# eyedealism/flexible-LLM-sharding

Measured on AMD Instinct MI355X. Metric: tokens/sec + peak GPU mem, Llama-2-70B layer_num_per_shard=1 at 1/2/4/8 MI355X, higher is better.
Workload: dtype fp16

## Files before the change

csrc/include/fls.h:

```cpp
#pragma once
#include <stdint.h>
#include <stddef.h>

#ifdef __cplusplus
extern "C" {
#endif

typedef void* fls_stream_t;

int   fls_rt_version(void);
void* fls_pinned_alloc(uint64_t bytes);
int   fls_pinned_free(void* p);
void* fls_host_device_ptr(void* p);
int   fls_pinned_register(void* p, uint64_t bytes);
int   fls_pinned_unregister(void* p);
int   fls_memcpy_async(void* dst, const void* src, uint64_t bytes, int kind, fls_stream_t s);
int64_t fls_pread_into(const char* path, uint64_t offset, uint64_t bytes, void* dst, int nthreads);
int64_t fls_pwrite_from(const char* path, uint64_t offset, uint64_t bytes, const void* src,
                        int nthreads, int truncate);
int   fls_gather_blocks(void* dst, const void* src, uint64_t block_bytes, const int64_t* src_block,
                        int64_t n_blocks, int nthreads);
void* fls_st_open(const char* path);
int   fls_st_count(void* h);
int   fls_st_info(void* h, int i, char* name, int name_cap, char* dtype, int dtype_cap,
// ... 31 lines not shown
             const float* sin_t, int rope_cols, int head_dim, const void* bias, const float* rscale,
             float alpha, float* ss, int ss_ld, void* ws, uint64_t ws_bytes,
             fls_stream_t s);
int fls_row_stat(const void* x, int ldx, int rows, int H, float eps, float* rstd, fls_stream_t s);
int fls_row_ss(const void* x, int ldx, int rows, int H, float* ss, int ss_ld, fls_stream_t s);
int fls_rstd_from_ss(const float* ss, int ss_ld, int nparts, int rows, int H, float eps, float* rstd,
                     fls_stream_t s);
int fls_argmax_rows(const void* x, int ld, int rows, int V, int* out, fls_stream_t s);
int fls_row_rstd(const void* x, int ldx, const int* row_idx, int rows, int H, float eps, float* rstd,
                 fls_stream_t s);
int fls_fold_norm(void* w, int ldw, int N, int K, const void* gamma, fls_stream_t s);
int fls_copy_d2d(void* dst, const void* src, uint64_t bytes, int mode, int blocks, fls_stream_t s);
int fls_copy_rows(const void* x, int ldx, const int* src_idx, void* y, int ldy, const int* dst_idx, int rows, int H,
                  fls_stream_t s);
int fls_gemm_set_splitk(int on);
int fls_gemm_set_row_chunk(int rows);
int fls_moe_route(const void* logits, int ldl, int T, int E, int k, int norm, int round16, int* ids, float* w,
                  fls_stream_t s);
int fls_moe_router_route(const void* h, int ldh, const void* wr, int ldw, int T, int H, int E, int k, int norm,
                         int round16, int* ids, float* w, fls_stream_t s);
int fls_moe_plan_scratch(int n, int E);
int fls_moe_plan(const int* ids, int n, int k, int E, int* offs, int* tiles, int* rows, int* dest, int* bhist,
                 fls_stream_t s);
int fls_moe_gemm(const void* A, const void* W, void* C, int M_bound, int N, int K, int lda, int ldw, int ldc, int epi,
                 const int* tiles, const int* offs, const int* rows, int n_groups, long long wstride, int a_rows,
                 fls_stream_t s);
int fls_moe_combine(const void* y, int ldy, const int* ids, const int* dest, const float* w, void* x, int ldx, int T,
                    int k, int H, const void* sh, int ldsh, fls_stream_t s);
int fls_gemm_set_order(int order);
int fls_gemm_set_mid_bn(int bn);
int fls_gemm_set_mid_waves(int waves);
int fls_gemm_set_mid_rows(int rows);
int fls_gemm_set_mid(int on);
int fls_attention_set_hpb(int hpb);
int fls_attention_set_split(int ns);
int fls_attention_set_persistent(int on);
int fls_attention(const void* qkv, void* out, const int* work, int n_items, int n_q_heads,
                  int n_kv_heads, int head_dim, int ld_qkv, int ld_out, float scale, const void* kv0,
                  int ld_kv0, const int* seg_lo, int q_block, const int* work2, const int* r2win,
                  void* ws, unsigned long long ws_bytes, int n_rows, fls_stream_t s);
int fls_attention_window(const void* qkv, void* out, const int* work, int n_items, int n_q_heads,
                         int n_kv_heads, int head_dim, int ld_qkv, int ld_out, float scale, const void* kv0,
                         int ld_kv0, const int* seg_lo, int q_block, const int* work2, const int* r2win,
                         void* ws, unsigned long long ws_bytes, int n_rows, const int* r0_lo,
                         const int* r0_item, fls_stream_t s);
int fls_headnorm_rope(void* x, int ldx, int rows, int n_q, int n_k, const void* qn, const void* kn, const int* pos,
                      const float* cos_t, const float* sin_t, int hd, float eps, fls_stream_t s);
int fls_rmsnorm(const void* x, const void* w, void* y, const int* row_idx, int rows, int H,
                int ldx, int ldy, float eps, fls_stream_t s);
int fls_embed(const int* ids, const void* table, void* out, int T, int H, int V, float scale, fls_stream_t s);
int fls_softmax_rows(const void* logits, void* probs, int rows, int V, float inv_scale, fls_stream_t s);
int fls_logprob_rows(const void* logits, int ld, int rows, int V, const int* targets, float inv_scale, float* out,
                     fls_stream_t s);
int fls_sample_rows(const void* probs, int ld, int rows, int V, const uint32_t* table, const uint64_t* draws,
                    int top_k, int P, int* out, fls_stream_t s);
int fls_topk_rows(const void* probs, int ld, int rows, int V, int K, int* ids, void* vals, const int* picked,
                  void* picked_vals, fls_stream_t s);
int fls_verify_rows(const void* probs, int ld, int rows, int V, const int* row_start, int n_sfx, const int* draft,
                    int* tok, int* accept, int* keep, int* n_kept, fls_stream_t s);
int fls_pool_rows(const void* x, int ld, int n_src, int H, const int* row_idx, int n_list, const int* seg_start,
                  int n_seg, int D, int normalize, float* out, fls_stream_t s);
int fls_cast_f16(void* dst, const void* src, int src_dtype, uint64_t n, fls_stream_t s);
int fls_dequant_fp8(void* region, uint64_t n, const float* scale, int kind, uint64_t cols, fls_stream_t s);
int fls_dequant_fp8_launches(uint64_t n);
int fls_dequant_fp8_tail(void);
int fls_dequant_int4(void* region, uint64_t n, uint64_t group, int scale_dtype, fls_stream_t s);
// ... 12 lines not shown
```

csrc/kernels/gemm.hip:

```cpp
#include "gemm_v10.h"

namespace {

template <int EPI>
__global__ __launch_bounds__(256) void gemm_nt_generic(const half_t* __restrict__ A, const half_t* __restrict__ W,
                                                     half_t* __restrict__ C, int M, int N, int K, int lda, int ldw,
                                                     int ldc, Epi ep) {
  const int lane = threadIdx.x & 63, wave = threadIdx.x >> 6;
  const int fr = lane & 15, grp = lane >> 4;
  const int m0 = blockIdx.x * 32;
  const bool rope128 = EPI == FLS_EPI_ROPE;
  const int gbase = blockIdx.y * 256 + (wave >> 1) * 128;
  int ncol[4];
#pragma unroll
  for (int t = 0; t < 4; ++t) ncol[t] = gbase + sub_col(rope128, wave & 1, t);
  floatx4 acc[2][4];
#pragma unroll
  for (int u = 0; u < 2; ++u)
#pragma unroll
    for (int t = 0; t < 4; ++t) acc[u][t] = floatx4{0.f, 0.f, 0.f, 0.f};
  for (int k0 = 0; k0 < K; k0 += 32) {
    half8 wf[4], xf[2];
    const int kb = k0 + grp * 8;
#pragma unroll
// ... 478 lines not shown
    FLS_CHECK_LAUNCH();
    ss_partials(C, ldc, M, N, ep, s);
    FLS_CHECK_LAUNCH();
    return 0;
  }
  const int n_chunks = (M + ROW_CHUNK - 1) / ROW_CHUNK;
  const int step = ((M + n_chunks - 1) / n_chunks + BM - 1) / BM * BM;
  if (M > ROW_CHUNK && (size_t)(step / BM) * (N / BN) >= 256) {
    for (int r0 = 0; r0 < M; r0 += step) {
      Epi e = ep;
      if (e.pos) e.pos += r0;
      if (e.R) e.R += (size_t)r0 * e.ldr;
      if (e.ss) e.ss += (size_t)r0 * e.ss_ld;
      if (e.rs) e.rs += r0;
      const int rc = launch<EPI>(A + (size_t)r0 * lda, W, C + (size_t)r0 * ldc, min(step, M - r0), N, K, lda, ldw,
                                 ldc, e, s, ws, ws_bytes);
      if (rc) return rc;
    }
    return 0;
  }
  const int tiles = (int)tiles256;
  const int tiles_m = (M + BM - 1) / BM, tiles_n = N / BN;
  int order = g_order;
  if (order == 0) order = auto_order(tiles_m, tiles_n);
  Epi e = ep;
  e.order = order;
  launch_main<EPI>(tiles, A, W, C, M, N, K, lda, ldw, ldc, e, s);
  FLS_CHECK_LAUNCH();
  return 0;
}

}

extern "C" int fls_kernels_version(void) { return 40; }

extern "C" int fls_gemm_set_order(int order) {
  const int old = g_order;
  g_order = order;
  return old;
}

extern "C" int fls_gemm_set_skinny(int mode, int blocks) {
  const int old = g_skinny;
  g_skinny = mode < 0 ? 0 : mode > 2 ? 2 : mode;
  g_skinny_blocks = blocks > 0 ? blocks : 0;
  return old;
}

extern "C" int fls_gemm_set_skinny_bn(int bn) {
  const int old = g_skinny_bn;
  g_skinny_bn = bn == 128 || bn == 256 ? bn : 0;
  return old;
}

extern "C" int fls_gemm_set_splitk(int on) {
  const int old = g_splitk;
  g_splitk = on ? 1 : 0;
  return old;
}

extern "C" int fls_gemm_set_row_chunk(int rows) {
  const int old = ROW_CHUNK;
  ROW_CHUNK = rows > 0 ? rows : (1 << 30);
  return old;
}

extern "C" int fls_row_ss(const void* x, int ldx, int rows, int H, float* ss, int ss_ld, fls_stream_t s) {
// ... 84 lines not shown
```

csrc/kernels/gemm_v10.h:

```cpp
#pragma once
#include "common.h"
#include "fls.h"

#include <cstdlib>
#include <type_traits>

namespace {


constexpr int BM = 256, BN = 256, BK = 64;
constexpr int EPI_ROPE64 = 4;
constexpr int EPI_F32 = 6;
constexpr bool is_rope(int epi) { return epi == FLS_EPI_ROPE || epi == EPI_ROPE64; }
constexpr int BUF = 65536;
constexpr int WIMG = 32768;

struct Epi {
  const half_t* R;
  int ldr;
  const int* pos;
  const float* cos_t;
  const float* sin_t;
  int rope_cols;
  int head_dim;
  const half_t* bias;
  int gu_rows;
  int order;
  const int* g_tiles;
  const int* g_offs;
  const int* g_rows;
  long long g_wstride;
  int g_n;
  int ksplit;
  int kslice;
  long long part_stride;
  const float* rs = nullptr;
  float alpha = 1.f;
  float* ss = nullptr;
  int ss_ld = 0;
  int row_exact = 0;
};

__device__ __forceinline__ float row_sum_4groups(float v) {
// ... 203 lines not shown
    return;
  } else {
    const int off = 4 * grp;
    const int woff = wide_off(grp);
    if constexpr (EPI == FLS_EPI_SWIGLU) {
#pragma unroll
      for (int u = 0; u < U; ++u) {
        const int m = mrow0 + u * 16;
        const float s = ep.rs ? ep.rs[min(m, M - 1)] : 1.f;
        half4 o[4];
#pragma unroll
        for (int p = 0; p < 4; ++p)
#pragma unroll
          for (int r = 0; r < 4; ++r) o[p][r] = (half_t)(silu(acc[u][2 * p][r] * s) * (acc[u][2 * p + 1][r] * s));
#pragma unroll
        for (int p = 0; p < 4; p += 2) {
          const uint4 v = wide_pair(o[p], o[p + 1]);
          if (m < M && (!LO || m >= mlo)) *(uint4*)(C + (size_t)m * ldc + ncol0 / 2 + p * 16 + woff) = v;
        }
      }
      return;
    } else {
      half4 ba[4], bb[4];
#pragma unroll
      for (int p = 0; p < 4; ++p) {
        if (ep.bias) {
          ba[p] = *(const half4*)(ep.bias + ncol0 + p * 32 + off);
          bb[p] = *(const half4*)(ep.bias + ncol0 + p * 32 + off + 16);
        } else {
          ba[p] = half4{0, 0, 0, 0};
          bb[p] = half4{0, 0, 0, 0};
        }
      }
      uint4 rw[2][4];
      auto load = [&](int u, int sl) {
        if constexpr (EPI == FLS_EPI_RESID) {
          const int m = min(mrow0 + u * 16, M - 1);
          const half_t* rp = ep.R + (size_t)m * ep.ldr + ncol0 + woff;
#pragma unroll
          for (int p = 0; p < 4; ++p) rw[sl][p] = *(const uint4*)(rp + p * 32);
        }
      };
      float* const ssp = EPI == FLS_EPI_RESID ? ep.ss : nullptr;
      auto body = [&](auto has_bias) {
        load(0, 0);
#pragma unroll
        for (int u = 0; u < U; ++u) {
          const int sl = u & 1;
          if (u + 1 < U) load(u + 1, sl ^ 1);
          asm volatile("" ::: "memory");
          const int m = mrow0 + u * 16;
          const float s = ep.rs ? ep.rs[min(m, M - 1)] : 1.f;
          float sq = 0.f;
#pragma unroll
          for (int p = 0; p < 4; ++p) {
            floatx4 a = acc[u][2 * p] * s, b = acc[u][2 * p + 1] * s;
            if constexpr (decltype(has_bias)::value) {
#pragma unroll
              for (int r = 0; r < 4; ++r) { a[r] += (float)ba[p][r]; b[r] += (float)bb[p][r]; }
            }
            if constexpr (EPI == FLS_EPI_RESID) {
              half4 ra, rb;
              unwide_pair(rw[sl][p], ra, rb);
#pragma unroll
              for (int r = 0; r < 4; ++r) { a[r] = a[r] * ep.alpha + (float)ra[r]; b[r] = b[r] * ep.alpha + (float)rb[r]; }
            }
            half4 oa, ob;
#pragma unroll
            for (int r = 0; r < 4; ++r) { oa[r] = (half_t)a[r]; ob[r] = (half_t)b[r]; }
            if constexpr (EPI == FLS_EPI_RESID) {
              if (ssp) sq = ss_accum_pair(sq, oa, ob);
            }
            const uint4 v = wide_pair(oa, ob);
            if (m < M && (!LO || m >= mlo)) *(uint4*)(C + (size_t)m * ldc + ncol0 + p * 32 + woff) = v;
          }
          if constexpr (EPI == FLS_EPI_RESID) {
            if (ssp) {
              sq = row_sum_4groups(sq);
              if (grp == 0 && m < M && (!LO || m >= mlo)) ssp[(size_t)m * ep.ss_ld + (ncol0 >> 7)] = sq;
            }
          }
        }
// ... 239 lines not shown
```

csrc/kernels/gemm_v11.hip:

```cpp
#include "gemm_v10.h"


namespace {
namespace v11 {
constexpr int TM = 384, TN = 256, TK = 64;
constexpr int X01_0 = 0, X01_STG = 32768;
constexpr int X2_0 = 65536, X2_STG = 16384;
constexpr int W_0 = 98304, W_STG = 32768;
constexpr int LDS_BYTES = 163840;
}

__device__ __forceinline__ void mfma_acc_v_ordered(floatx4& c, const half8& a, const half8& b) {
  asm volatile("v_mfma_f32_16x16x32_f16 %0, %1, %2, %0" : "+v"(c) : "v"(a), "v"(b) : "memory");
}

template <int EPI>
__global__ __launch_bounds__(256, 1) void gemm_nt_v11(const half_t* __restrict__ A, const half_t* __restrict__ W,
                                                    half_t* __restrict__ C, int M, int N, int K, int lda, int ldw,
                                                    int ldc, Epi ep) {
  using namespace v11;
  extern __shared__ __attribute__((aligned(16))) char smem[];
  const int tid = threadIdx.x;
  const int lane = tid & 63;
  const int wave = __builtin_amdgcn_readfirstlane(tid >> 6);

  const int nwg = gridDim.x;
  int bid = blockIdx.x;
  {
    const int q = nwg >> 3, r = nwg & 7, xcd = bid & 7, loc = bid >> 3;
    bid = (xcd < r ? xcd * (q + 1) : r * (q + 1) + (xcd - r) * q) + loc;
  }
  const int tiles_m = (M + TM - 1) / TM;
  const int tiles_n = N / TN;
  const int2 tmn = tile_of(bid, tiles_m, tiles_n, ep.order);
  const int mlo = tmn.x * TM;
  const int m0 = min(mlo, M - TM);
  const int n0 = tmn.y * TN;

  const int lr = lane >> 3;
  const int lc = (lane & 7) ^ lr;
  const unsigned xl = (unsigned)(lr * lda + lc * 8) * 2u;
  const unsigned wl = (unsigned)(lr * ldw + lc * 8) * 2u;
  const char* Ab = (const char*)(A + (size_t)m0 * lda);
  const char* Wb = (const char*)(W + (size_t)(EPI == FLS_EPI_SWIGLU ? n0 / 2 : n0) * ldw);
  auto rsrc = [](const char* base, bool live) {
    return __builtin_amdgcn_make_buffer_rsrc(const_cast<char*>(base), (short)0, live ? -1 : 0, 0x00020000);
  };
  int xlds_p[3][4];
  unsigned xso[3][4];
#pragma unroll
  for (int j = 0; j < 3; ++j)
#pragma unroll
    for (int i = 0; i < 4; ++i) {
      const int p = 4 * wave + i;
      const int src_row = (p >> 3) * 192 + j * 64 + (p & 7) * 8;
      xlds_p[j][i] = j < 2 ? X01_0 + ((p >> 3) * 128 + j * 64 + (p & 7) * 8) * 128
                           : X2_0 + ((p >> 3) * 64 + (p & 7) * 8) * 128;
      xso[j][i] = (unsigned)(src_row * lda) * 2u;
    }
  unsigned wso[8];
#pragma unroll
  for (int i = 0; i < 8; ++i) {
    const int l = (8 * wave + i) * 8;
    const int pr = EPI == FLS_EPI_SWIGLU ? ((l >> 4) & 1) * ep.gu_rows + (l >> 5) * 16 + (l & 15) : l;
    wso[i] = (unsigned)(pr * ldw) * 2u;
  }
#define V11_DMA_X(rs, buf, j, i, k0)                                                               \
  __builtin_amdgcn_raw_ptr_buffer_load_lds(                                                        \
      rs, (LDS_AS void*)(smem + xlds_p[j][i] + (buf) * ((j) < 2 ? X01_STG : X2_STG)), 16, xl,      \
      xso[j][i] + (unsigned)(k0) * 2u, 0, 0)
#define V11_DMA_W(rs, buf, i, k0)                                                                  \
  __builtin_amdgcn_raw_ptr_buffer_load_lds(rs, (LDS_AS void*)(smem + W_0 + (buf) * W_STG + (8 * wave + (i)) * 1024), \
                                           16, wl, wso[i] + (unsigned)(k0) * 2u, 0, 0)

  const int wm = wave >> 1, wn = wave & 1;
  const int fr = lane & 15, grp = lane >> 4;
  const int sw = fr & 7;
  const int cs0 = ((0 + grp) ^ sw) << 4;
  const int cs1 = ((4 + grp) ^ sw) << 4;
  const int xrow = X01_0 + (wm * 128 + fr) * 128;
  const int x2row = X2_0 + (wm * 64 + fr) * 128;
  const int wrow = W_0 + (wn * 128 + fr) * 128;

  floatx4 acc[8][8], accv[4][8];
#pragma unroll
  for (int u = 0; u < 8; ++u)
#pragma unroll
    for (int t = 0; t < 8; ++t) acc[u][t] = floatx4{0.f, 0.f, 0.f, 0.f};
#pragma unroll
  for (int u = 0; u < 4; ++u)
#pragma unroll
    for (int t = 0; t < 8; ++t) accv[u][t] = floatx4{0.f, 0.f, 0.f, 0.f};
  half8 xf[12], wf[8];
#define V11_FENCE_ACC()                                                                            \
  _Pragma("unroll") for (int u_ = 0; u_ < 8; ++u_)                                                \
  _Pragma("unroll") for (int t_ = 0; t_ < 8; ++t_) asm volatile("" : "+a"(acc[u_][t_]));          \
  _Pragma("unroll") for (int u_ = 0; u_ < 4; ++u_)                                                \
  _Pragma("unroll") for (int t_ = 0; t_ < 8; ++t_) asm volatile("" : "+v"(accv[u_][t_]));
  V11_FENCE_ACC();
  asm volatile("s_nop 7\n\ts_nop 7" ::: "memory");

  const char* const bx01_0 = smem + xrow + cs0;
  const char* const bx01_1 = smem + xrow + cs1;
  const char* const bx2_0 = smem + x2row + cs0;
  const char* const bx2_1 = smem + x2row + cs1;
  const char* const bw_0 = smem + wrow + cs0;
  const char* const bw_1 = smem + wrow + cs1;
#define V11_RX(f, buf, s)                                                                          \
  xf[f] = (f) < 8 ? *(const half8*)(((s) ? bx01_1 : bx01_0) + (buf) * X01_STG + (f) * 2048)        \
                  : *(const half8*)(((s) ? bx2_1 : bx2_0) + (buf) * X2_STG + ((f) - 8) * 2048)
#define V11_RW(t, buf, s) wf[t] = *(const half8*)(((s) ? bw_1 : bw_0) + (buf) * W_STG + (t) * 2048)
#define V11_MFMA(u, t)                                                                             \
  do {                                                                                            \
    if ((u) < 8) mfma_acc_inplace_ordered(acc[(u) & 7][t], wf[t], xf[u]);                         \
    else mfma_acc_v_ordered(accv[(u) & 3][t], wf[t], xf[u]);                                      \
  } while (0)
#define V11_DMA_AT(i_, ND)                                                                         \
  ((ND) == 2 ? ((i_) == 9 ? 0 : (i_) == 21 ? 1 : -1)                                              \
   : (ND) == 4 ? ((i_) == 7 ? 0 : (i_) == 13 ? 1 : (i_) == 19 ? 2 : (i_) == 25 ? 3 : -1)          \
   : ((i_) == 5 ? 0 : (i_) == 9 ? 1 : (i_) == 13 ? 2 : (i_) == 17 ? 3 : (i_) == 21 ? 4 : (i_) == 25 ? 5 : -1))
#define V11_DMAS(i_, DMA_STMT, ND)                                                                 \
  {                                                                                               \
    const int d_ = V11_DMA_AT(i_, ND);                                                            \
    if (d_ >= 0) { DMA_STMT(d_); }                                                                \
  }
#define V11_SYNC(LGK, VMC)                                                                         \
  {                                                                                               \
    __builtin_amdgcn_s_waitcnt(0xC07F | ((LGK) << 8));                                            \
    asm volatile("s_waitcnt vmcnt(" #VMC ")" ::: "memory");                                       \
    __builtin_amdgcn_s_barrier();                                                                 \
  }

#define V11_PHASE_A(cbuf, cs, nbuf, ns, DMA_STMT, ND)                                             \
  _Pragma("unroll") for (int i_ = 0; i_ < 32; ++i_) {                                             \
    const int t_ = i_ >> 2, u_ = i_ & 3;                                                          \
    V11_MFMA(u_, t_);                                                                             \
    if (i_ == 1) V11_RX(8, cbuf, cs);                                                             \
    if (i_ == 3) V11_RX(9, cbuf, cs);                                                             \
    if (i_ >= 28) V11_RX(u_, nbuf, ns);                                                           \
    V11_DMAS(i_, DMA_STMT, ND);                                                                   \
  }
#define V11_PHASE_B(cbuf, cs, nbuf, ns, DMA_STMT, ND)                                             \
  _Pragma("unroll") for (int i_ = 0; i_ < 32; ++i_) {                                             \
    const int u_ = 4 + (i_ >> 3), t_ = i_ & 7;                                                    \
    V11_MFMA(u_, t_);                                                                             \
    if (i_ == 1) V11_RX(10, cbuf, cs);                                                            \
    if (i_ == 3) V11_RX(11, cbuf, cs);                                                            \
    if ((i_ & 7) == 7) V11_RX(u_, nbuf, ns);                                                      \
    V11_DMAS(i_, DMA_STMT, ND);                                                                   \
  }
#define V11_PHASE_C(nbuf, ns, DMA_STMT, ND)                                                       \
  _Pragma("unroll") for (int i_ = 0; i_ < 32; ++i_) {                                             \
    const int t_ = i_ >> 2, u_ = 8 + (i_ & 3);                                                    \
    V11_MFMA(u_, t_);                                                                             \
    if ((i_ & 3) == 3) V11_RW(t_, nbuf, ns);                                                      \
    V11_DMAS(i_, DMA_STMT, ND);                                                                   \
  }

  const int nk = K / TK;
  const __amdgpu_buffer_rsrc_t rA = rsrc(Ab, true), rW = rsrc(Wb, true);
  const __amdgpu_buffer_rsrc_t rZA = rsrc(Ab, false), rZW = rsrc(Wb, false);
  {
    const int k1 = min(1, nk - 1) * TK;
#pragma unroll
    for (int i = 0; i < 4; ++i) V11_DMA_X(rA, 0, 0, i, 0);
#pragma unroll
    for (int i = 0; i < 4; ++i) V11_DMA_X(rA, 0, 1, i, 0);
#pragma unroll
    for (int i = 0; i < 8; ++i) V11_DMA_W(rW, 0, i, 0);
#pragma unroll
    for (int i = 0; i < 4; ++i) V11_DMA_X(rA, 0, 2, i, 0);
#pragma unroll
    for (int i = 0; i < 4; ++i) V11_DMA_X(rA, 1, 0, i, k1);
#pragma unroll
    for (int i = 0; i < 4; ++i) V11_DMA_X(rA, 1, 1, i, k1);
#pragma unroll
    for (int i = 0; i < 4; ++i) V11_DMA_W(rW, 1, i, k1);
  }
  asm volatile("s_waitcnt vmcnt(12)" ::: "memory");
  __builtin_amdgcn_s_barrier();
#pragma unroll
  for (int u = 0; u < 8; ++u) V11_RX(u, 0, 0);
#pragma unroll
  for (int t = 0; t < 8; ++t) V11_RW(t, 0, 0);

  for (int kt = 0; kt < nk; kt += 2) {
    const int k1 = min(kt + 1, nk - 1) * TK, k2 = min(kt + 2, nk - 1) * TK, k3 = min(kt + 3, nk - 1) * TK;
    const __amdgpu_buffer_rsrc_t rX1 = kt + 1 < nk ? rA : rZA;
    const __amdgpu_buffer_rsrc_t rX2 = kt + 2 < nk ? rA : rZA, rW2 = kt + 2 < nk ? rW : rZW;
    const __amdgpu_buffer_rsrc_t rX3 = kt + 3 < nk ? rA : rZA, rW3 = kt + 3 < nk ? rW : rZW;
    const __amdgpu_buffer_rsrc_t rW1 = kt + 1 < nk ? rW : rZW;
#define V11_TILE(B, rXn, rWn, kn, rXf, rWf, kf)                                                    \
  {                                                                                               \
    auto dX2 = [&](int d) { V11_DMA_X(rXn, (B) ^ 1, 2, d, kn); };                                 \
    auto dWhi = [&](int d) { V11_DMA_W(rWn, (B) ^ 1, d + 4, kn); };                               \
    auto dX0a = [&](int d) { V11_DMA_X(rXf, B, 0, d, kf); };                                      \
    auto dX0b = [&](int d) { V11_DMA_X(rXf, B, 0, d + 2, kf); };                                  \
    auto dX1 = [&](int d) { V11_DMA_X(rXf, B, 1, d, kf); };                                       \
    auto dWlo = [&](int d) { V11_DMA_W(rWf, B, d, kf); };                                         \
    V11_PHASE_A(B, 0, B, 1, dX2, 4);                                                   \
    V11_PHASE_B(B, 0, B, 1, dWhi, 4);                                                  \
    V11_SYNC(6, 16);                                                                    \
    V11_PHASE_C(B, 1, dX0a, 2);                                                        \
    V11_PHASE_A(B, 1, (B) ^ 1, 0, dX0b, 2);                                            \
    V11_SYNC(6, 4);                                                                     \
    V11_PHASE_B(B, 1, (B) ^ 1, 0, dX1, 4);                                             \
    V11_PHASE_C((B) ^ 1, 0, dWlo, 4);                                                  \
    V11_SYNC(8, 12);                                                                    \
  }
    V11_TILE(0, rX1, rW1, k1, rX2, rW2, k2);
    V11_TILE(1, rX2, rW2, k2, rX3, rW3, k3);
#undef V11_TILE
  }
  asm volatile("s_waitcnt vmcnt(0)" ::: "memory");
  asm volatile("s_nop 7\n\ts_nop 7\n\ts_nop 7" ::: "memory");
  V11_FENCE_ACC();
#undef V11_FENCE_ACC
#undef V11_RX
#undef V11_RW
#undef V11_MFMA
#undef V11_DMA_AT
#undef V11_DMAS
#undef V11_SYNC
#undef V11_PHASE_A
#undef V11_PHASE_B
#undef V11_PHASE_C
#undef V11_DMA_X
#undef V11_DMA_W

  const int mrow = m0 + wm * 192 + fr, ncol = n0 + wn * 128;
  epilogue_quadrant<EPI, 4, true>(C, ldc, M, mrow + 128, ncol, grp, accv, ep, mlo);
  epilogue_quadrant<EPI, 8, true>(C, ldc, M, mrow, ncol, grp, acc, ep, mlo);
}

int g_v11 = 1;
int g_v11_cost = 145;

bool v11_pays(int M, int N) {
  using namespace v11;
  const long t11 = (long)((M + TM - 1) / TM) * (N / TN);
  const long r11 = (t11 + 255) / 256;
  const int n_chunks = M > 16384 ? (M + 16383) / 16384 : 1;
  const int step = ((M + n_chunks - 1) / n_chunks + 255) / 256 * 256;
  long r10 = 0;
  for (int r0 = 0; r0 < M; r0 += step) {
    const long t10 = (long)((min(step, M - r0) + 255) / 256) * (N / 256);
    r10 += (t10 + 255) / 256;
  }
  return r11 * g_v11_cost <= r10 * 100;
}

template <int EPI>
int launch_v11(const half_t* A, const half_t* W, half_t* C, int M, int N, int K, int lda, int ldw, int ldc, Epi ep,
               hipStream_t s) {
  using namespace v11;
  static bool attr = false;
  if (!attr) {
    (void)hipFuncSetAttribute((const void*)gemm_nt_v11<EPI>, hipFuncAttributeMaxDynamicSharedMemorySize, LDS_BYTES);
    attr = true;
  }
  const int tiles_m = (M + TM - 1) / TM, tiles_n = N / TN;
  ep.order = auto_order(tiles_m, tiles_n);
  hipLaunchKernelGGL((gemm_nt_v11<EPI>), dim3(tiles_m * tiles_n), dim3(256), LDS_BYTES, s, A, W, C, M, N, K, lda, ldw,
                     ldc, ep);
  FLS_CHECK_LAUNCH();
  return 0;
}

}

extern "C" int fls_gemm_set_v11(int mode) {
  const int old = g_v11;
  g_v11 = mode < 0 ? 0 : mode > 2 ? 2 : mode;
  return old;
}

extern "C" int fls_gemm_v11_pays(int M, int N) { return v11_pays(M, N) ? 1 : 0; }

extern "C" int fls_gemm_set_v11_cost(int cost) {
  const int old = g_v11_cost;
  if (cost > 0) g_v11_cost = cost;
  return old;
}

extern "C" int fls_gemm_v11_try(const void* A, const void* W, void* C, const void* R, int M, int N, int K, int lda,
                                int ldw, int ldc, int ldr, int epi, const int* pos, const float* cos_t,
                                const float* sin_t, int rope_cols, int head_dim, const void* bias,
                                const float* rscale, float alpha, float* ss, int ss_ld, fls_stream_t s) {
  using namespace v11;
  if (!g_v11 || M < TM || N % TN || K % TK || (K / TK) % 2 || lda % 8 || ldw % 8) return 0;
  if (g_v11 == 1) {
    if ((size_t)((M + TM - 1) / TM) * (N / TN) < 256 || !v11_pays(M, N)) return 0;
  }
  if ((size_t)M * lda * 2 >= (1ull << 32)) return 0;
  if (epi == FLS_EPI_SWIGLU && (size_t)(N / 2 + TN) * ldw * 2 >= (1ull << 32)) return 0;
  if ((size_t)N * ldw * 2 >= (1ull << 32)) return 0;
  if (ldc % 8 || ((uintptr_t)C & 15)) return 0;
  if (epi == FLS_EPI_RESID && (ldr % 8 || ((uintptr_t)R & 15))) return 0;
  Epi ep{(const half_t*)R, ldr, pos, cos_t, sin_t, rope_cols, head_dim, (const half_t*)bias, N / 2, 0,
         nullptr, nullptr, nullptr, 0, 0};
  ep.rs = rscale;
  ep.alpha = alpha;
  ep.ss = ss;
  ep.ss_ld = ss_ld;
  auto a = (const half_t*)A;
  auto w = (const half_t*)W;
  auto c = (half_t*)C;
  auto st = (hipStream_t)s;
// ... 14 lines not shown
```

flexible_llm_sharding_amd/_native/__init__.py:

```python
from __future__ import annotations

import ctypes
import os
import threading

HERE = os.path.dirname(os.path.abspath(__file__))
_KERNELS = os.path.join(HERE, "libfls_kernels.so")
_RUNTIME = os.path.join(HERE, "libfls_runtime.so")
_COMM = os.path.join(HERE, "libfls_comm.so")

_lock = threading.Lock()
_libs = {}

c_void_p, c_int, c_int64, c_uint64, c_float, c_char_p = (
    ctypes.c_void_p, ctypes.c_int, ctypes.c_int64, ctypes.c_uint64, ctypes.c_float, ctypes.c_char_p)


def _bind(lib, name, restype, *argtypes):
    f = getattr(lib, name)
    f.restype = restype
    f.argtypes = list(argtypes)


def _load_runtime():
# ... 2 lines not shown
    _bind(lib, "fls_pinned_alloc", c_void_p, c_uint64)
    _bind(lib, "fls_pinned_free", c_int, c_void_p)
    _bind(lib, "fls_pinned_register", c_int, c_void_p, c_uint64)
    _bind(lib, "fls_host_device_ptr", c_void_p, c_void_p)
    _bind(lib, "fls_pinned_unregister", c_int, c_void_p)
    _bind(lib, "fls_memcpy_async", c_int, c_void_p, c_void_p, c_uint64, c_int, c_void_p)
    _bind(lib, "fls_pread_into", c_int64, c_char_p, c_uint64, c_uint64, c_void_p, c_int)
    _bind(lib, "fls_pwrite_from", c_int64, c_char_p, c_uint64, c_uint64, c_void_p, c_int, c_int)
    _bind(lib, "fls_gather_blocks", c_int, c_void_p, c_void_p, c_uint64, c_void_p, c_int64, c_int)
    _bind(lib, "fls_st_open", c_void_p, c_char_p)
    _bind(lib, "fls_st_count", c_int, c_void_p)
    _bind(lib, "fls_st_info", c_int, c_void_p, c_int, c_char_p, c_int, c_char_p, c_int,
          c_void_p, c_void_p, c_void_p, c_void_p)
    _bind(lib, "fls_st_data_offset", c_uint64, c_void_p)
    _bind(lib, "fls_st_close", None, c_void_p)
    _bind(lib, "fls_mem_info", c_int, c_void_p, c_void_p)
    _bind(lib, "fls_device_alloc", c_void_p, c_int, c_uint64)
    _bind(lib, "fls_device_free", c_int, c_int, c_void_p)
    _bind(lib, "fls_streamer_create", c_void_p, c_int, c_uint64, c_int, c_int, c_int)
    _bind(lib, "fls_streamer_pinned_bytes", c_uint64, c_void_p)
    _bind(lib, "fls_streamer_load", c_int64, c_void_p, c_char_p, c_void_p, c_int, c_void_p, c_void_p)
    _bind(lib, "fls_stream_read_host", c_int64, c_char_p, c_void_p, c_int, c_void_p, c_int)
    _bind(lib, "fls_streamer_stats", c_int, c_void_p, c_void_p, c_void_p, c_void_p, c_void_p, c_void_p)
    _bind(lib, "fls_streamer_destroy", None, c_void_p)
    _bind(lib, "fls_f32_to_f16", None, c_void_p, c_void_p, c_uint64)
    return lib


class Piece(ctypes.Structure):
    _fields_ = [("file_off", ctypes.c_uint64), ("nbytes", ctypes.c_uint64), ("dst_off", ctypes.c_uint64),
                ("kind", ctypes.c_int32), ("pad", ctypes.c_int32)]


KERNELS_ABI = 40


def _load_kernels(path: str = _KERNELS):
    lib = ctypes.CDLL(path)
    _bind(lib, "fls_kernels_version", c_int)
    if lib.fls_kernels_version() != KERNELS_ABI:
        raise RuntimeError(f"{path} is a stale build (ABI {lib.fls_kernels_version()} != {KERNELS_ABI}); "
                           "rebuild with python -m flexible_llm_sharding_amd._native.build")
    _bind(lib, "fls_gemm", c_int, c_void_p, c_void_p, c_void_p, c_void_p, c_int, c_int, c_int,
          c_int, c_int, c_int, c_int, c_int, c_void_p, c_void_p, c_void_p, c_int, c_int, c_void_p, c_void_p,
          c_float, c_void_p, c_int, c_void_p, c_uint64, c_void_p)
    _bind(lib, "fls_rstd_from_ss", c_int, c_void_p, c_int, c_int, c_int, c_int, c_float, c_void_p, c_void_p)
    _bind(lib, "fls_row_ss", c_int, c_void_p, c_int, c_int, c_int, c_void_p, c_int, c_void_p)
    _bind(lib, "fls_row_stat", c_int, c_void_p, c_int, c_int, c_int, c_float, c_void_p, c_void_p)
    _bind(lib, "fls_argmax_rows", c_int, c_void_p, c_int, c_int, c_int, c_void_p, c_void_p)
    _bind(lib, "fls_row_rstd", c_int, c_void_p, c_int, c_void_p, c_int, c_int, c_float, c_void_p, c_void_p)
    _bind(lib, "fls_fold_norm", c_int, c_void_p, c_int, c_int, c_int, c_void_p, c_void_p)
    _bind(lib, "fls_copy_d2d", c_int, c_void_p, c_void_p, c_uint64, c_int, c_int, c_void_p)
    _bind(lib, "fls_copy_rows", c_int, c_void_p, c_int, c_void_p, c_void_p, c_int, c_void_p, c_int, c_int, c_void_p)
    _bind(lib, "fls_gemm_set_splitk", c_int, c_int)
    _bind(lib, "fls_gemm_set_row_chunk", c_int, c_int)
    _bind(lib, "fls_gemm_set_mid", c_int, c_int)
    _bind(lib, "fls_gemm_set_mid_bn", c_int, c_int)
    _bind(lib, "fls_gemm_set_mid_waves", c_int, c_int)
    _bind(lib, "fls_gemm_set_mid_rows", c_int, c_int)
    _bind(lib, "fls_moe_route", c_int, c_void_p, c_int, c_int, c_int, c_int, c_int, c_int, c_void_p, c_void_p,
          c_void_p)
    _bind(lib, "fls_moe_router_route", c_int, c_void_p, c_int, c_void_p, c_int, c_int, c_int, c_int, c_int, c_int,
          c_int, c_void_p, c_void_p, c_void_p)
    _bind(lib, "fls_moe_plan_scratch", c_int, c_int, c_int)
    _bind(lib, "fls_moe_plan", c_int, c_void_p, c_int, c_int, c_int, c_void_p, c_void_p, c_void_p, c_void_p, c_void_p,
          c_void_p)
    _bind(lib, "fls_moe_gemm", c_int, c_void_p, c_void_p, c_void_p, c_int, c_int, c_int, c_int, c_int, c_int, c_int,
          c_void_p, c_void_p, c_void_p, c_int, ctypes.c_longlong, c_int, c_void_p)
    _bind(lib, "fls_moe_combine", c_int, c_void_p, c_int, c_void_p, c_void_p, c_void_p, c_void_p, c_int, c_int,
          c_int, c_int, c_void_p, c_int, c_void_p)
    _bind(lib, "fls_gemm_set_order", c_int, c_int)
    _bind(lib, "fls_gemm_set_v11", c_int, c_int)
    _bind(lib, "fls_gemm_set_v11_cost", c_int, c_int)
    _bind(lib, "fls_gemm_v11_pays", c_int, c_int, c_int)
    _bind(lib, "fls_gemm_set_skinny", c_int, c_int, c_int)
    _bind(lib, "fls_gemm_set_skinny_bn", c_int, c_int)
    _bind(lib, "fls_attention_set_hpb", c_int, c_int)
    _bind(lib, "fls_attention_set_split", c_int, c_int)
    _bind(lib, "fls_attention_set_persistent", c_int, c_int)
    _bind(lib, "fls_attention", c_int, c_void_p, c_void_p, c_void_p, c_int, c_int, c_int, c_int,
          c_int, c_int, c_float, c_void_p, c_int, c_void_p, c_int, c_void_p, c_void_p, c_void_p, c_uint64, c_int,
          c_void_p)
    _bind(lib, "fls_attention_window", c_int, c_void_p, c_void_p, c_void_p, c_int, c_int, c_int, c_int,
          c_int, c_int, c_float, c_void_p, c_int, c_void_p, c_int, c_void_p, c_void_p, c_void_p, c_uint64, c_int,
          c_void_p, c_void_p, c_void_p)
    _bind(lib, "fls_rmsnorm", c_int, c_void_p, c_void_p, c_void_p, c_void_p, c_int, c_int, c_int,
          c_int, c_float, c_void_p)
    _bind(lib, "fls_headnorm_rope", c_int, c_void_p, c_int, c_int, c_int, c_int, c_void_p, c_void_p, c_void_p,
          c_void_p, c_void_p, c_int, c_float, c_void_p)
    _bind(lib, "fls_embed", c_int, c_void_p, c_void_p, c_void_p, c_int, c_int, c_int, c_float, c_void_p)
    _bind(lib, "fls_softmax_rows", c_int, c_void_p, c_void_p, c_int, c_int, c_float, c_void_p)
    _bind(lib, "fls_logprob_rows", c_int, c_void_p, c_int, c_int, c_int, c_void_p, c_float, c_void_p, c_void_p)
    _bind(lib, "fls_sample_rows", c_int, c_void_p, c_int, c_int, c_int, c_void_p, c_void_p, c_int, c_int, c_void_p,
          c_void_p)
    _bind(lib, "fls_topk_rows", c_int, c_void_p, c_int, c_int, c_int, c_int, c_void_p, c_void_p, c_void_p, c_void_p,
          c_void_p)
    _bind(lib, "fls_verify_rows", c_int, c_void_p, c_int, c_int, c_int, c_void_p, c_int, c_void_p, c_void_p, c_void_p,
          c_void_p, c_void_p, c_void_p)
    _bind(lib, "fls_pool_rows", c_int, c_void_p, c_int, c_int, c_int, c_void_p, c_int, c_void_p, c_int, c_int, c_int,
          c_void_p, c_void_p)
    _bind(lib, "fls_cast_f16", c_int, c_void_p, c_void_p, c_int, c_uint64, c_void_p)
    _bind(lib, "fls_dequant_fp8", c_int, c_void_p, c_uint64, c_void_p, c_int, c_uint64, c_void_p)
    _bind(lib, "fls_dequant_fp8_launches", c_int, c_uint64)
    _bind(lib, "fls_dequant_fp8_tail", c_int)
    _bind(lib, "fls_dequant_int4", c_int, c_void_p, c_uint64, c_uint64, c_int, c_void_p)
    _bind(lib, "fls_dequant_int4_launches", c_int, c_uint64, c_uint64, c_int)
    _bind(lib, "fls_dequant_int4_tail", c_int)
# ... 55 lines not shown
```

Measured before the change: 10210.

## Make v11 GEMM persistent with cross-tile prefetch and deeper residual load pipeline

Turns the v11 GEMM into a persistent kernel: the grid is capped at the CU count (rounded to a multiple of 8), and each workgroup loops over tiles. The first K-slices of the next tile are prefetched during the tail of the current one. Per-tile setup is recomputed from the kernarg segment to keep register pressure down. It also deepens the residual-epilogue load pipeline from 2 to a configurable depth of up to 8. This adds register pressure and more complex control flow, and may cause load imbalance when the tile count is not a multiple of the grid.

Result: faster. 10320, median of 6 (+1.1%).

```diff
diff --git a/csrc/include/fls.h b/csrc/include/fls.h
--- a/csrc/include/fls.h
+++ b/csrc/include/fls.h
@@ -87,6 +87,8 @@
 int fls_gemm_set_mid_waves(int waves);
 int fls_gemm_set_mid_rows(int rows);
 int fls_gemm_set_mid(int on);
+int fls_gemm_set_v11_grid(int g);
+int fls_gemm_v11_grid(int M, int N, int cus);
 int fls_attention_set_hpb(int hpb);
 int fls_attention_set_split(int ns);
 int fls_attention_set_persistent(int on);
diff --git a/csrc/kernels/gemm.hip b/csrc/kernels/gemm.hip
--- a/csrc/kernels/gemm.hip
+++ b/csrc/kernels/gemm.hip
@@ -534,7 +534,7 @@
 
 }
 
-extern "C" int fls_kernels_version(void) { return 40; }
+extern "C" int fls_kernels_version(void) { return 41; }
 
 extern "C" int fls_gemm_set_order(int order) {
   const int old = g_order;
diff --git a/csrc/kernels/gemm_v10.h b/csrc/kernels/gemm_v10.h
--- a/csrc/kernels/gemm_v10.h
+++ b/csrc/kernels/gemm_v10.h
@@ -9,6 +9,15 @@
 
 
 constexpr int BM = 256, BN = 256, BK = 64;
+#ifndef V10_RESID_DEPTH
+#define V10_RESID_DEPTH 8
+#endif
+#ifndef V11_RESID_DEPTH
+#define V11_RESID_DEPTH 8
+#endif
+#ifndef V11_RESID_DEPTH4
+#define V11_RESID_DEPTH4 2
+#endif
 constexpr int EPI_ROPE64 = 4;
 constexpr int EPI_F32 = 6;
 constexpr bool is_rope(int epi) { return epi == FLS_EPI_ROPE || epi == EPI_ROPE64; }
@@ -278,7 +287,10 @@
           bb[p] = half4{0, 0, 0, 0};
         }
       }
-      uint4 rw[2][4];
+      constexpr int D = EPI != FLS_EPI_RESID ? 2
+                        : (LO && U == 8) ? V11_RESID_DEPTH : (LO && U == 4) ? V11_RESID_DEPTH4 : V10_RESID_DEPTH;
+      static_assert(D >= 2 && D <= (U > 2 ? U : 2), "residual-load depth");
+      uint4 rw[D][4];
       auto load = [&](int u, int sl) {
         if constexpr (EPI == FLS_EPI_RESID) {
           const int m = min(mrow0 + u * 16, M - 1);
@@ -289,11 +301,12 @@
       };
       float* const ssp = EPI == FLS_EPI_RESID ? ep.ss : nullptr;
       auto body = [&](auto has_bias) {
-        load(0, 0);
+#pragma unroll
+        for (int u = 0; u < D - 1 && u < U; ++u) load(u, u);
 #pragma unroll
         for (int u = 0; u < U; ++u) {
-          const int sl = u & 1;
-          if (u + 1 < U) load(u + 1, sl ^ 1);
+          const int sl = u % D;
+          if (u + D - 1 < U) load(u + D - 1, (u + D - 1) % D);
           asm volatile("" ::: "memory");
           const int m = mrow0 + u * 16;
           const float s = ep.rs ? ep.rs[min(m, M - 1)] : 1.f;
diff --git a/csrc/kernels/gemm_v11.hip b/csrc/kernels/gemm_v11.hip
--- a/csrc/kernels/gemm_v11.hip
+++ b/csrc/kernels/gemm_v11.hip
@@ -20,92 +20,106 @@
                                                     int ldc, Epi ep) {
   using namespace v11;
   extern __shared__ __attribute__((aligned(16))) char smem[];
-  const int tid = threadIdx.x;
-  const int lane = tid & 63;
-  const int wave = __builtin_amdgcn_readfirstlane(tid >> 6);
-
-  const int nwg = gridDim.x;
-  int bid = blockIdx.x;
-  {
-    const int q = nwg >> 3, r = nwg & 7, xcd = bid & 7, loc = bid >> 3;
-    bid = (xcd < r ? xcd * (q + 1) : r * (q + 1) + (xcd - r) * q) + loc;
-  }
-  const int tiles_m = (M + TM - 1) / TM;
-  const int tiles_n = N / TN;
-  const int2 tmn = tile_of(bid, tiles_m, tiles_n, ep.order);
-  const int mlo = tmn.x * TM;
-  const int m0 = min(mlo, M - TM);
-  const int n0 = tmn.y * TN;
-
-  const int lr = lane >> 3;
-  const int lc = (lane & 7) ^ lr;
-  const unsigned xl = (unsigned)(lr * lda + lc * 8) * 2u;
-  const unsigned wl = (unsigned)(lr * ldw + lc * 8) * 2u;
-  const char* Ab = (const char*)(A + (size_t)m0 * lda);
-  const char* Wb = (const char*)(W + (size_t)(EPI == FLS_EPI_SWIGLU ? n0 / 2 : n0) * ldw);
-  auto rsrc = [](const char* base, bool live) {
-    return __builtin_amdgcn_make_buffer_rsrc(const_cast<char*>(base), (short)0, live ? -1 : 0, 0x00020000);
-  };
-  int xlds_p[3][4];
-  unsigned xso[3][4];
-#pragma unroll
-  for (int j = 0; j < 3; ++j)
-#pragma unroll
-    for (int i = 0; i < 4; ++i) {
-      const int p = 4 * wave + i;
-      const int src_row = (p >> 3) * 192 + j * 64 + (p & 7) * 8;
-      xlds_p[j][i] = j < 2 ? X01_0 + ((p >> 3) * 128 + j * 64 + (p & 7) * 8) * 128
-                           : X2_0 + ((p >> 3) * 64 + (p & 7) * 8) * 128;
-      xso[j][i] = (unsigned)(src_row * lda) * 2u;
-    }
-  unsigned wso[8];
-#pragma unroll
-  for (int i = 0; i < 8; ++i) {
-    const int l = (8 * wave + i) * 8;
-    const int pr = EPI == FLS_EPI_SWIGLU ? ((l >> 4) & 1) * ep.gu_rows + (l >> 5) * 16 + (l & 15) : l;
-    wso[i] = (unsigned)(pr * ldw) * 2u;
-  }
+  const int wave0 = __builtin_amdgcn_readfirstlane((int)threadIdx.x >> 6);
+  int wave, wm, wn, fr, grp;
+  struct KArgs {
+    const half_t* A;
+    const half_t* W;
+    half_t* C;
+    int M, N, K, lda, ldw, ldc;
+    Epi ep;
+  };
+  static_assert(offsetof(KArgs, ldc) == 44 && offsetof(KArgs, ep) == 48, "KArgs must mirror the kernel's parameters");
+  auto kargs = []() {
+    auto p = __builtin_amdgcn_kernarg_segment_ptr();
+    asm volatile("" : "+s"(p));
+    return (const __attribute__((address_space(4))) KArgs*)p;
+  };
+
+  const int nwg = ((kargs()->M + TM - 1) / TM) * (kargs()->N / TN);
+  auto tile_at = [&](int v, int& mlo_, int& n0_) {
+    const auto* ka = kargs();
+    const int tiles_m = (ka->M + TM - 1) / TM, tiles_n = ka->N / TN;
+    const int q = nwg >> 3, r = nwg & 7, xcd = v & 7, loc = v >> 3;
+    const int bid = (xcd < r ? xcd * (q + 1) : r * (q + 1) + (xcd - r) * q) + loc;
+    const int2 tmn = tile_of(bid, tiles_m, tiles_n, ka->ep.order);
+    mlo_ = tmn.x * TM;
+    n0_ = tmn.y * TN;
+  };
+  int vt = blockIdx.x;
+  int mlo, n0;
+  tile_at(vt, mlo, n0);
+
+  unsigned xl, wl;
+  auto a_off = [&](int mlo_) {
+    const auto* ka = kargs();
+    return (unsigned)(min(mlo_, ka->M - TM) * ka->lda) * 2u;
+  };
+  auto w_off = [&](int n0_) {
+    const auto* ka = kargs();
+    return (unsigned)((EPI == FLS_EPI_SWIGLU ? n0_ / 2 : n0_) * ka->ldw) * 2u;
+  };
+  auto rsrc = [](const half_t* base, bool live) {
+    return __builtin_amdgcn_make_buffer_rsrc(const_cast<half_t*>(base), (short)0, live ? -1 : 0, 0x00020000);
+  };
+  int xb01, xb2, wb;
+  unsigned xs0, xstep, ws0, wstep, wgu;
+  const char *bx01_0, *bx01_1, *bx2_0, *bx2_1, *bw_0, *bw_1;
+  auto setup = [&]() {
+    unsigned ones = ~0u;
+    int wv = wave0;
+    asm volatile("" : "+s"(ones), "+s"(wv));
+    const int lane = __builtin_amdgcn_mbcnt_hi(ones, __builtin_amdgcn_mbcnt_lo(ones, 0u));
+    wave = wv;
+    const auto* ka = kargs();
+    const int lda = ka->lda, ldw = ka->ldw;
+    const int lr = lane >> 3;
+    const int lc = (lane & 7) ^ lr;
+    xl = (unsigned)(lr * lda + lc * 8) * 2u;
+    wl = (unsigned)(lr * ldw + lc * 8) * 2u;
+    xb01 = X01_0 + ((wave >> 1) * 128 + (wave & 1) * 32) * 128;
+    xb2 = X2_0 + ((wave >> 1) * 64 + (wave & 1) * 32) * 128;
+    wb = W_0 + 8 * wave * 1024;
+    xs0 = (unsigned)(((wave >> 1) * 192 + (wave & 1) * 32) * lda) * 2u;
+    xstep = (unsigned)(8 * lda) * 2u;
+    ws0 = (unsigned)((EPI == FLS_EPI_SWIGLU ? 32 : 64) * wave * ldw) * 2u;
+    wstep = (unsigned)(8 * ldw) * 2u;
+    wgu = EPI == FLS_EPI_SWIGLU ? (unsigned)(ka->ep.gu_rows * ldw) * 2u : 0u;
+    wm = wave >> 1, wn = wave & 1;
+    fr = lane & 15, grp = lane >> 4;
+    const int sw = fr & 7;
+    const int cs0 = ((0 + grp) ^ sw) << 4;
+    const int cs1 = ((4 + grp) ^ sw) << 4;
+    const int xrow = X01_0 + (wm * 128 + fr) * 128;
+    const int x2row = X2_0 + (wm * 64 + fr) * 128;
+    const int wrow = W_0 + (wn * 128 + fr) * 128;
+    bx01_0 = smem + xrow + cs0;
+    bx01_1 = smem + xrow + cs1;
+    bx2_0 = smem + x2row + cs0;
+    bx2_1 = smem + x2row + cs1;
+    bw_0 = smem + wrow + cs0;
+    bw_1 = smem + wrow + cs1;
+  };
+  setup();
 #define V11_DMA_X(rs, buf, j, i, k0)                                                               \
   __builtin_amdgcn_raw_ptr_buffer_load_lds(                                                        \
-      rs, (LDS_AS void*)(smem + xlds_p[j][i] + (buf) * ((j) < 2 ? X01_STG : X2_STG)), 16, xl,      \
-      xso[j][i] + (unsigned)(k0) * 2u, 0, 0)
+      rs,                                                                                          \
+      (LDS_AS void*)(smem + ((j) < 2 ? xb01 + (j) * 8192 + (buf) * X01_STG : xb2 + (buf) * X2_STG) + (i) * 1024), \
+      16, xl, xs0 + (unsigned)(8 * (j) + (i)) * xstep + (k0), 0, 0)
+#define V11_WC(i) (EPI == FLS_EPI_SWIGLU ? ((i) >> 2) * 2 + ((i) & 1) : (i))
 #define V11_DMA_W(rs, buf, i, k0)                                                                  \
-  __builtin_amdgcn_raw_ptr_buffer_load_lds(rs, (LDS_AS void*)(smem + W_0 + (buf) * W_STG + (8 * wave + (i)) * 1024), \
-                                           16, wl, wso[i] + (unsigned)(k0) * 2u, 0, 0)
-
-  const int wm = wave >> 1, wn = wave & 1;
-  const int fr = lane & 15, grp = lane >> 4;
-  const int sw = fr & 7;
-  const int cs0 = ((0 + grp) ^ sw) << 4;
-  const int cs1 = ((4 + grp) ^ sw) << 4;
-  const int xrow = X01_0 + (wm * 128 + fr) * 128;
-  const int x2row = X2_0 + (wm * 64 + fr) * 128;
-  const int wrow = W_0 + (wn * 128 + fr) * 128;
+  __builtin_amdgcn_raw_ptr_buffer_load_lds(                                                        \
+      rs, (LDS_AS void*)(smem + wb + (buf) * W_STG + (i) * 1024), 16, wl,                          \
+      ws0 + (unsigned)V11_WC(i) * wstep + (EPI == FLS_EPI_SWIGLU && (((i) >> 1) & 1) ? wgu : 0u) + (k0), 0, 0)
 
   floatx4 acc[8][8], accv[4][8];
-#pragma unroll
-  for (int u = 0; u < 8; ++u)
-#pragma unroll
-    for (int t = 0; t < 8; ++t) acc[u][t] = floatx4{0.f, 0.f, 0.f, 0.f};
-#pragma unroll
-  for (int u = 0; u < 4; ++u)
-#pragma unroll
-    for (int t = 0; t < 8; ++t) accv[u][t] = floatx4{0.f, 0.f, 0.f, 0.f};
   half8 xf[12], wf[8];
 #define V11_FENCE_ACC()                                                                            \
   _Pragma("unroll") for (int u_ = 0; u_ < 8; ++u_)                                                \
   _Pragma("unroll") for (int t_ = 0; t_ < 8; ++t_) asm volatile("" : "+a"(acc[u_][t_]));          \
   _Pragma("unroll") for (int u_ = 0; u_ < 4; ++u_)                                                \
   _Pragma("unroll") for (int t_ = 0; t_ < 8; ++t_) asm volatile("" : "+v"(accv[u_][t_]));
-  V11_FENCE_ACC();
-  asm volatile("s_nop 7\n\ts_nop 7" ::: "memory");
-
-  const char* const bx01_0 = smem + xrow + cs0;
-  const char* const bx01_1 = smem + xrow + cs1;
-  const char* const bx2_0 = smem + x2row + cs0;
-  const char* const bx2_1 = smem + x2row + cs1;
-  const char* const bw_0 = smem + wrow + cs0;
-  const char* const bw_1 = smem + wrow + cs1;
+
 #define V11_RX(f, buf, s)                                                                          \
   xf[f] = (f) < 8 ? *(const half8*)(((s) ? bx01_1 : bx01_0) + (buf) * X01_STG + (f) * 2048)        \
                   : *(const half8*)(((s) ? bx2_1 : bx2_0) + (buf) * X2_STG + ((f) - 8) * 2048)
@@ -157,47 +171,76 @@
     V11_DMAS(i_, DMA_STMT, ND);                                                                   \
   }
 
-  const int nk = K / TK;
-  const __amdgpu_buffer_rsrc_t rA = rsrc(Ab, true), rW = rsrc(Wb, true);
-  const __amdgpu_buffer_rsrc_t rZA = rsrc(Ab, false), rZW = rsrc(Wb, false);
+  const int nk = kargs()->K / TK;
   {
-    const int k1 = min(1, nk - 1) * TK;
-#pragma unroll
-    for (int i = 0; i < 4; ++i) V11_DMA_X(rA, 0, 0, i, 0);
-#pragma unroll
-    for (int i = 0; i < 4; ++i) V11_DMA_X(rA, 0, 1, i, 0);
-#pragma unroll
-    for (int i = 0; i < 8; ++i) V11_DMA_W(rW, 0, i, 0);
-#pragma unroll
-    for (int i = 0; i < 4; ++i) V11_DMA_X(rA, 0, 2, i, 0);
-#pragma unroll
-    for (int i = 0; i < 4; ++i) V11_DMA_X(rA, 1, 0, i, k1);
-#pragma unroll
-    for (int i = 0; i < 4; ++i) V11_DMA_X(rA, 1, 1, i, k1);
-#pragma unroll
-    for (int i = 0; i < 4; ++i) V11_DMA_W(rW, 1, i, k1);
+    const __amdgpu_buffer_rsrc_t rA = rsrc(kargs()->A, true), rW = rsrc(kargs()->W, true);
+    const unsigned a0 = a_off(mlo), w0 = w_off(n0), a1 = a0 + TK * 2, w1 = w0 + TK * 2;
+#pragma unroll
+    for (int i = 0; i < 4; ++i) V11_DMA_X(rA, 0, 0, i, a0);
+#pragma unroll
+    for (int i = 0; i < 4; ++i) V11_DMA_X(rA, 0, 1, i, a0);
+#pragma unroll
+    for (int i = 0; i < 8; ++i) V11_DMA_W(rW, 0, i, w0);
+#pragma unroll
+    for (int i = 0; i < 4; ++i) V11_DMA_X(rA, 0, 2, i, a0);
+#pragma unroll
+    for (int i = 0; i < 4; ++i) V11_DMA_X(rA, 1, 0, i, a1);
+#pragma unroll
+    for (int i = 0; i < 4; ++i) V11_DMA_X(rA, 1, 1, i, a1);
+#pragma unroll
+    for (int i = 0; i < 4; ++i) V11_DMA_W(rW, 1, i, w1);
   }
   asm volatile("s_waitcnt vmcnt(12)" ::: "memory");
   __builtin_amdgcn_s_barrier();
+
+  for (;;) {
+  setup();
+  const int vnext = vt + (int)gridDim.x;
+  const bool more = vnext < nwg;
+  int mlo_n = mlo, n0_n = n0;
+  if (more) tile_at(vnext, mlo_n, n0_n);
+  const __amdgpu_buffer_rsrc_t rA = rsrc(kargs()->A, true), rW = rsrc(kargs()->W, true);
+  const __amdgpu_buffer_rsrc_t rNA = rsrc(kargs()->A, more), rNW = rsrc(kargs()->W, more);
+  const unsigned ao = a_off(mlo), wo = w_off(n0), ao_n = a_off(mlo_n), wo_n = w_off(n0_n);
+
+  float zero = 0.f;
+  asm volatile("" : "+v"(zero));
+#pragma unroll
+  for (int u = 0; u < 8; ++u)
+#pragma unroll
+    for (int t = 0; t < 8; ++t) acc[u][t] = floatx4{zero, zero, zero, zero};
+#pragma unroll
+  for (int u = 0; u < 4; ++u)
+#pragma unroll
+    for (int t = 0; t < 8; ++t) accv[u][t] = floatx4{zero, zero, zero, zero};
+  V11_FENCE_ACC();
+  asm volatile("s_nop 7\n\ts_nop 7" ::: "memory");
 #pragma unroll
   for (int u = 0; u < 8; ++u) V11_RX(u, 0, 0);
 #pragma unroll
   for (int t = 0; t < 8; ++t) V11_RW(t, 0, 0);
+  if constexpr (EPI == FLS_EPI_RESID) {
+    __builtin_amdgcn_s_waitcnt(0x0F70);
+  }
 
   for (int kt = 0; kt < nk; kt += 2) {
-    const int k1 = min(kt + 1, nk - 1) * TK, k2 = min(kt + 2, nk - 1) * TK, k3 = min(kt + 3, nk - 1) * TK;
-    const __amdgpu_buffer_rsrc_t rX1 = kt + 1 < nk ? rA : rZA;
-    const __amdgpu_buffer_rsrc_t rX2 = kt + 2 < nk ? rA : rZA, rW2 = kt + 2 < nk ? rW : rZW;
-    const __amdgpu_buffer_rsrc_t rX3 = kt + 3 < nk ? rA : rZA, rW3 = kt + 3 < nk ? rW : rZW;
-    const __amdgpu_buffer_rsrc_t rW1 = kt + 1 < nk ? rW : rZW;
-#define V11_TILE(B, rXn, rWn, kn, rXf, rWf, kf)                                                    \
+    const bool in2 = kt + 2 < nk;
+    const unsigned ak1 = ao + (kt + 1) * TK * 2, wk1 = wo + (kt + 1) * TK * 2;
+    const unsigned ak2 = in2 ? ao + (kt + 2) * TK * 2 : ao_n, wk2 = in2 ? wo + (kt + 2) * TK * 2 : wo_n;
+    const unsigned ak3 = ak2 + TK * 2, wk3 = wk2 + TK * 2;
+    const __amdgpu_buffer_rsrc_t rX1 = rA;
+    const __amdgpu_buffer_rsrc_t rX2 = in2 ? rA : rNA, rW2 = in2 ? rW : rNW;
+    const __amdgpu_buffer_rsrc_t rX3 = in2 ? rA : rNA, rW3 = in2 ? rW : rNW;
+    const __amdgpu_buffer_rsrc_t rW1 = rW;
+#define V11_TILE(B, rXn, rWn, akn, wkn, rXf, rWf, akf, wkf)                                                  \
   {                                                                                               \
-    auto dX2 = [&](int d) { V11_DMA_X(rXn, (B) ^ 1, 2, d, kn); };                                 \
-    auto dWhi = [&](int d) { V11_DMA_W(rWn, (B) ^ 1, d + 4, kn); };                               \
-    auto dX0a = [&](int d) { V11_DMA_X(rXf, B, 0, d, kf); };                                      \
-    auto dX0b = [&](int d) { V11_DMA_X(rXf, B, 0, d + 2, kf); };                                  \
-    auto dX1 = [&](int d) { V11_DMA_X(rXf, B, 1, d, kf); };                                       \
-    auto dWlo = [&](int d) { V11_DMA_W(rWf, B, d, kf); };                                         \
+    asm volatile("" : "+s"(xstep), "+s"(wstep), "+s"(xb01), "+s"(xb2), "+s"(wb));                   \
+    auto dX2 = [&](int d) { V11_DMA_X(rXn, (B) ^ 1, 2, d, akn); };                                \
+    auto dWhi = [&](int d) { V11_DMA_W(rWn, (B) ^ 1, d + 4, wkn); };                              \
+    auto dX0a = [&](int d) { V11_DMA_X(rXf, B, 0, d, akf); };                                     \
+    auto dX0b = [&](int d) { V11_DMA_X(rXf, B, 0, d + 2, akf); };                                 \
+    auto dX1 = [&](int d) { V11_DMA_X(rXf, B, 1, d, akf); };                                      \
+    auto dWlo = [&](int d) { V11_DMA_W(rWf, B, d, wkf); };                                        \
     V11_PHASE_A(B, 0, B, 1, dX2, 4);                                                   \
     V11_PHASE_B(B, 0, B, 1, dWhi, 4);                                                  \
     V11_SYNC(6, 16);                                                                    \
@@ -208,8 +251,8 @@
     V11_PHASE_C((B) ^ 1, 0, dWlo, 4);                                                  \
     V11_SYNC(8, 12);                                                                    \
   }
-    V11_TILE(0, rX1, rW1, k1, rX2, rW2, k2);
-    V11_TILE(1, rX2, rW2, k2, rX3, rW3, k3);
+    V11_TILE(0, rX1, rW1, ak1, wk1, rX2, rW2, ak2, wk2);
+    V11_TILE(1, rX2, rW2, ak2, wk2, rX3, rW3, ak3, wk3);
 #undef V11_TILE
   }
   asm volatile("s_waitcnt vmcnt(0)" ::: "memory");
@@ -227,10 +270,24 @@
 #undef V11_PHASE_C
 #undef V11_DMA_X
 #undef V11_DMA_W
-
-  const int mrow = m0 + wm * 192 + fr, ncol = n0 + wn * 128;
-  epilogue_quadrant<EPI, 4, true>(C, ldc, M, mrow + 128, ncol, grp, accv, ep, mlo);
-  epilogue_quadrant<EPI, 8, true>(C, ldc, M, mrow, ncol, grp, acc, ep, mlo);
+#undef V11_WC
+
+  {
+    setup();
+    const auto* ka = kargs();
+    Epi epe;
+    __builtin_memcpy(&epe, &ka->ep, sizeof(Epi));
+    half_t* const Ce = ka->C;
+    const int Me = ka->M, ldce = ka->ldc;
+    const int mrow = min(mlo, Me - TM) + wm * 192 + fr, ncol = n0 + wn * 128;
+    epilogue_quadrant<EPI, 4, true>(Ce, ldce, Me, mrow + 128, ncol, grp, accv, epe, mlo);
+    epilogue_quadrant<EPI, 8, true>(Ce, ldce, Me, mrow, ncol, grp, acc, epe, mlo);
+  }
+  if (!more) break;
+  vt = vnext;
+  mlo = mlo_n;
+  n0 = n0_n;
+  }
 }
 
 int g_v11 = 1;
@@ -250,6 +307,29 @@
   return r11 * g_v11_cost <= r10 * 100;
 }
 
+int g_v11_grid = 0;
+
+int v11_grid(int M, int N, int cus) {
+  using namespace v11;
+  const long tiles = (long)((M + TM - 1) / TM) * (N / TN);
+  if (g_v11_grid < 0) return (int)tiles;
+  long g = cus >= 8 ? cus - cus % 8 : cus > 0 ? cus : 1;
+  if (g_v11_grid > 0 && g_v11_grid < g) g = g_v11_grid;
+  return (int)(g < tiles ? g : tiles);
+}
+
+int v11_cus() {
+  static int cus[64];
+  int dev = 0;
+  if (hipGetDevice(&dev) != hipSuccess || dev < 0 || dev >= 64) dev = 0;
+  if (!cus[dev]) {
+    int n = 0;
+    if (hipDeviceGetAttribute(&n, hipDeviceAttributeMultiprocessorCount, dev) != hipSuccess || n <= 0) n = 256;
+    cus[dev] = n;
+  }
+  return cus[dev];
+}
+
 template <int EPI>
 int launch_v11(const half_t* A, const half_t* W, half_t* C, int M, int N, int K, int lda, int ldw, int ldc, Epi ep,
                hipStream_t s) {
@@ -261,8 +341,8 @@
   }
   const int tiles_m = (M + TM - 1) / TM, tiles_n = N / TN;
   ep.order = auto_order(tiles_m, tiles_n);
-  hipLaunchKernelGGL((gemm_nt_v11<EPI>), dim3(tiles_m * tiles_n), dim3(256), LDS_BYTES, s, A, W, C, M, N, K, lda, ldw,
-                     ldc, ep);
+  hipLaunchKernelGGL((gemm_nt_v11<EPI>), dim3(v11_grid(M, N, v11_cus())), dim3(256), LDS_BYTES, s, A, W, C, M, N, K,
+                     lda, ldw, ldc, ep);
   FLS_CHECK_LAUNCH();
   return 0;
 }
@@ -274,6 +354,14 @@
   g_v11 = mode < 0 ? 0 : mode > 2 ? 2 : mode;
   return old;
 }
+
+extern "C" int fls_gemm_set_v11_grid(int g) {
+  const int old = g_v11_grid;
+  g_v11_grid = g;
+  return old;
+}
+
+extern "C" int fls_gemm_v11_grid(int M, int N, int cus) { return v11_grid(M, N, cus); }
 
 extern "C" int fls_gemm_v11_pays(int M, int N) { return v11_pays(M, N) ? 1 : 0; }
 
diff --git a/flexible_llm_sharding_amd/_native/__init__.py b/flexible_llm_sharding_amd/_native/__init__.py
--- a/flexible_llm_sharding_amd/_native/__init__.py
+++ b/flexible_llm_sharding_amd/_native/__init__.py
@@ -58,7 +58,7 @@
                 ("kind", ctypes.c_int32), ("pad", ctypes.c_int32)]
 
 
-KERNELS_ABI = 40
+KERNELS_ABI = 41
 
 
 def _load_kernels(path: str = _KERNELS):
@@ -99,6 +99,8 @@
     _bind(lib, "fls_gemm_set_v11", c_int, c_int)
     _bind(lib, "fls_gemm_set_v11_cost", c_int, c_int)
     _bind(lib, "fls_gemm_v11_pays", c_int, c_int, c_int)
+    _bind(lib, "fls_gemm_set_v11_grid", c_int, c_int)
+    _bind(lib, "fls_gemm_v11_grid", c_int, c_int, c_int, c_int)
     _bind(lib, "fls_gemm_set_skinny", c_int, c_int, c_int)
     _bind(lib, "fls_gemm_set_skinny_bn", c_int, c_int)
     _bind(lib, "fls_attention_set_hpb", c_int, c_int)
```
